# PhiFEM/phiFEM

Hardware: AMD Instinct MI355X
Metric: assembled+solved DoF/s, 3D Poisson phi-FEM (tag+assemble+solve) (higher is better)
Workload: dtype f64

## Files before the change

include/phifem_hip.h:

```cpp
#ifndef PHIFEM_HIP_H
#define PHIFEM_HIP_H

#include <stdint.h>

#ifdef __cplusplus
extern "C" {
#endif

typedef struct phx_mesh phx_mesh;
typedef struct phx_system phx_system;

enum phx_status {
  PHX_OK = 0,
  PHX_ERR_VALUE = -1,
  PHX_ERR_NOT_IMPLEMENTED = -2,
  PHX_ERR_HIP = -3,
  PHX_ERR_PARTITION = -4,
  PHX_ERR_CAPACITY = -5,
  PHX_ERR_BREAKDOWN = -6,
  PHX_ERR_TIMEOUT = -7
};

enum phx_loc { PHX_HOST = 0, PHX_DEVICE = 1 };

// ... 42 lines not shown
                            int32_t *c2f, int32_t *f2c, int64_t *nf);

int phx_mesh_create(int gdim, int cell_type, int64_t nv, const double *coords, int64_t nc,
                    const int32_t *cells, int device, phx_mesh **out);

int phx_mesh_create_box(int gdim, const double *lo, const double *hi, const int64_t *n,
                        const int64_t *offset, const int64_t *n_global, int device,
                        phx_mesh **out);

int phx_mesh_set_slab_faces(phx_mesh *m, int lower_is_cut, int upper_is_cut);
int phx_mesh_destroy(phx_mesh *m);
int phx_mesh_edge_count(phx_mesh *m, int64_t *ne);
int phx_mesh_counts(const phx_mesh *m, int64_t *counts);
int phx_mesh_get_array(phx_mesh *m, int which, void *out, int loc);
int phx_mesh_stream(phx_mesh *m, uint64_t *stream);
int phx_mesh_synchronize(phx_mesh *m);
int phx_mesh_set_stream(phx_mesh *m, uint64_t stream);
enum phx_option {
  PHX_OPT_PROFILE_SPMV = 1,
  PHX_OPT_HAS_EXTERIOR = 2,
  PHX_OPT_SPMV_XCD_GROUP = 3,
  PHX_OPT_PRECOND = 5,
  PHX_OPT_EXPORT_CSR = 7,
  PHX_OPT_STRUCTURED = 8,
  PHX_OPT_DETERMINISTIC = 9,
  PHX_OPT_EL_COARSE = 10,
  PHX_OPT_STENCIL_PLANE_ROWS = 11,
  PHX_OPT_P2_COARSE = 12,
  PHX_OPT_BOX_TAGS = 13,
  PHX_OPT_MULTILEVEL = 14,
  PHX_OPT_ELWD_COARSE = 15,
  PHX_OPT_BOX_FACET_ROWS = 16,
  PHX_OPT_RED_SPMV = 17,
  PHX_OPT_ALLOW_EMPTY = 6,
  PHX_OPT_SPMV_VALUE_INDEX = 4
};
int phx_set_option(phx_mesh *m, int option, int64_t value);
int phx_box_poisson_solve(int device, const int *L, const double *h, int f32, double *f_host);
int phx_box_dst_bench(int device, const int *L, int f32, int reps, double *out_us3);
int phx_dense_inverse(int device, int64_t n, double *a_host, int *singular);
int phx_event_pair_overhead(phx_mesh *m, double *seconds);
int phx_mesh_tag_histogram(const phx_mesh *m, int64_t *cells4, int64_t *facets7);

int phx_tag_cells(phx_mesh *m, int phi_kind, const double *phi, int loc, int detection_degree,
                  int single_layer_cut, int *warn_zero_denominator);

int phx_tag_facets(phx_mesh *m, int phi_kind, const double *phi, int loc, int detection_degree);

int phx_overwrite_tags(phx_mesh *m, int entity_is_facet, int64_t n, const int32_t *indices,
                       const int32_t *values);
int phx_set_tags(phx_mesh *m, int entity_is_facet, const int32_t *values, int loc);

int phx_mesh_selection(phx_mesh *m, int which, int32_t *out, int64_t *count);
int phx_integration_entities(phx_mesh *m, int which, int32_t *out, int64_t *n_pairs);

int phx_submesh_create(phx_mesh *m, phx_mesh **sub);
int phx_submesh_maps(phx_mesh *sub, int32_t *c_map, int32_t *v_map);

int phx_partition_cells(phx_mesh *m, int nparts, const int32_t *weights, int32_t *part, int loc);
int phx_partition_layout(phx_mesh *m, int nparts, const int32_t *part, int rank, int32_t *owner, uint8_t *flags, int loc);
int phx_submesh_create_from_flags(phx_mesh *m, const uint8_t *flags, int loc, phx_mesh **sub);

int phx_mesh_refine(phx_mesh *m, phx_mesh **fine);
int phx_prolongate(phx_mesh *coarse, phx_mesh *fine, int degree, int ncomp, const double *in, int loc_in,
                   double *out, int loc_out);
int phx_refine_tables(int cell_type, int32_t *children, int *nchild, double *p2_weights);
// ... 34 lines not shown
int phx_system_update_rhs(phx_system *s, const double *phi_h, const double *f_h, const double *g_h,
                          const double *u_D, int loc);
int phx_assemble_diffusion_wd(phx_mesh *m, double pen_coef, double stab_coef, double reaction, const double *kappa_h,
                              const double *phi_h, const double *f_h, const double *g_h, const double *u_D, int loc,
                              phx_system **out);
int phx_system_destroy(phx_system *s);
int phx_system_info(const phx_system *s, int64_t *info);
int phx_system_export(phx_system *s, int64_t *rowptr, int32_t *col, double *val, double *rhs,
                      int64_t *dof);
int phx_system_export_sell(phx_system *s, int64_t *slice_ptr, int32_t *col, double *val, int32_t *rows);

enum phx_method { PHX_BICGSTAB_JACOBI = 0 };
int phx_solve(phx_system *s, int method, double rtol, int64_t max_iter, double *x, int loc,
              double *stats);
int phx_solve_from(phx_system *s, int method, double rtol, int64_t max_iter, const double *x0, double *x, int loc,
                   double *stats);

int phx_krylov_attach(phx_system *s, double *work, double *scal, const uint8_t *own);
int phx_krylov_precond_active(const phx_system *s, int *active);
int phx_precond_local_bbox(phx_system *s, int64_t *out6);
int phx_precond_setup_global(phx_system *s, const int64_t *bbox6, int nranks, int rank, const int64_t *zb,
                             int64_t *ncol);
int phx_precond_set_carry_buffers(phx_system *s, double *send, double *recv);
int phx_precond_dist_info(const phx_system *s, int64_t *out4);
int phx_krylov_precond_disable(phx_system *s);
int phx_precond_info(phx_system *s, double *out);
int phx_multilevel_setup(phx_system *s);
int phx_coarse_info(phx_system *s, double *out);
int phx_coarse_export(phx_system *s, int32_t *node_of, double *ainv);
int phx_coarse_apply(phx_system *s, const double *in, double *out, double *gc, double *zc, int loc);
int phx_krylov_identity_loop(const phx_system *s, int *on);
int phx_krylov_reduced_loop(const phx_system *s, int *on);
int phx_krylov_reduced_io(phx_system *s, int which, double *host, int64_t count, int put);
int phx_krylov_phase(phx_system *s, int phase);
int phx_krylov_finish(phx_system *s, double *x, int loc);
int phx_krylov_profile(phx_system *s, int reset, double *avg_seconds, int64_t *count);
int phx_system_get_perm(phx_system *s, int32_t *perm, int32_t *dof_u, int32_t *dof_p, int loc);

typedef struct phx_comm phx_comm;
int phx_comm_unique_id(void *out128);
int phx_comm_create(int nranks, int rank, const void *uid128, int device, phx_comm **out);
int phx_comm_destroy(phx_comm *c);
int phx_comm_library(char *out, int64_t len);
int phx_comm_overlap(const phx_comm *c, int *out);
int phx_solve_distributed(phx_system *s, phx_comm *c, int npeers, const int *peers,
                          const int64_t *counts, const int64_t *const *idx, double rtol,
                          int64_t max_iter, double *x, int loc, double *stats);
int phx_halo_selftest(phx_system *s, phx_comm *c, int npeers, const int *peers,
                      const int64_t *counts, const int64_t *const *idx, double *vec);

int phx_spmv(phx_system *s, const double *x, double *y, int loc);
int phx_reference_nodes(int gdim, int degree, double *bary, int *n_nodes);
int phx_cell_errors(phx_mesh *m, int ncomp, int degree_h, const double *u_h, const double *u_ref,
                    int64_t ncells, const int32_t *cell_list, int loc, double *l2_local,
                    double *h10_local, double *norms);
int phx_estimate_poisson_wd(phx_mesh *m, int degree, const double *u, const double *p, const double *phi,
                            const double *f, const double *u_D, int loc_in, double *eta2_parts, int loc_out,
                            double *sums3);
int phx_mark_dorfler(phx_mesh *m, int64_t n, const double *eta2, int loc_in, double theta, uint8_t *marked,
                     int loc_out, int64_t *n_marked);
int phx_recover_gradient(phx_mesh *m, int degree, int ncomp, const double *u, int loc_u, const uint8_t *cell_mask,
                         int loc_mask, double *grad, double *eta2, int loc_out, double *sum);

int phx_spmv_bench(phx_system *s, int reps, double *out);

int phx_last_timings(const phx_mesh *m, double *t);
// ... 6 lines not shown
```

phifem_amd/_lib.py:

```python
import ctypes as C
import os

_HERE = os.path.dirname(os.path.abspath(__file__))
LIB_PATH = os.path.join(_HERE, "libphifem_hip.so")

if not os.path.exists(LIB_PATH):
    raise ImportError(
        f"{LIB_PATH} is missing: build it with `python -c 'import __graft_entry__ as g; g.build()'` "
        "(or `make -C phifem_amd/csrc`).  phifem_amd has no CPU fallback.")

if os.environ.get("PHIFEM_NO_TORCH", "") != "1":
    try:
        import torch
    except ImportError:
        pass

lib = C.CDLL(LIB_PATH)

HOST, DEVICE = 0, 1
TRIANGLE, QUADRILATERAL, TETRAHEDRON = 0, 1, 2
CELL_TYPES = {"triangle": TRIANGLE, "quadrilateral": QUADRILATERAL, "tetrahedron": TETRAHEDRON}
CELL_NAMES = {v: k for k, v in CELL_TYPES.items()}
PHI_NODAL_P1, PHI_POINTS, PHI_QUADRIC = 0, 1, 2
(OPT_PROFILE_SPMV, OPT_HAS_EXTERIOR, OPT_SPMV_XCD_GROUP, OPT_SPMV_VALUE_INDEX, OPT_PRECOND, OPT_ALLOW_EMPTY,
 OPT_EXPORT_CSR, OPT_STRUCTURED, OPT_DETERMINISTIC, OPT_EL_COARSE, OPT_STENCIL_PLANE_ROWS, OPT_P2_COARSE,
 OPT_BOX_TAGS, OPT_MULTILEVEL, OPT_ELWD_COARSE, OPT_BOX_FACET_ROWS, OPT_RED_SPMV) = (
    1, 2, 3, 4, 5, 6, 7, 8, 9, 10, 11, 12, 13, 14, 15, 16, 17)
(ARR_COORDS, ARR_CELLS, ARR_C2F, ARR_F2C, ARR_CELL_TAGS, ARR_FACET_TAGS, ARR_BFACETS, ARR_C2E,
 ARR_EDGES, ARR_PARENT_CELLS, ARR_CHILD_NODES) = range(11)

OK, ERR_VALUE, ERR_NOT_IMPLEMENTED, ERR_HIP, ERR_PARTITION, ERR_CAPACITY, ERR_BREAKDOWN, ERR_TIMEOUT = (
    0, -1, -2, -3, -4, -5, -6, -7)

_vp, _i, _i64, _d = C.c_void_p, C.c_int, C.c_int64, C.c_double
_pi, _pi64, _pd = C.POINTER(C.c_int), C.POINTER(C.c_int64), C.POINTER(C.c_double)

SIGNATURES = {
    "phx_version": ([], _i),
    "phx_last_error": ([], C.c_char_p),
    "phx_device_count": ([_pi], _i),
    "phx_pool_release": ([], _i),
    "phx_pool_stats": ([_pi64, _pi64], _i),
    "phx_detection_points": ([_i, _i, _i, _vp, _pi64], _i),
    "phx_levelset_points_count": ([_vp, _i, _pi64], _i),
    "phx_levelset_eval_points": ([_vp, _i, _vp, _i, _vp], _i),
    "phx_detection_points_physical": ([_vp, _i, _vp], _i),
    "phx_lagrange_nodes": ([_i, _i, _vp, _pi64], _i),
    "phx_lagrange_tabulate": ([_i, _i, _i64, _vp, _vp], _i),
    "phx_levelset_eval_points_deg": ([_vp, _i, _i, _vp, _i, _vp], _i),
    "phx_lagrange_dof_points": ([_vp, _i, _vp], _i),
    "phx_topology_build_host": ([_i, _i64, _i64, _vp, _vp, _vp, _pi64], _i),
    "phx_mesh_create": ([_i, _i, _i64, _vp, _i64, _vp, _i, C.POINTER(_vp)], _i),
    "phx_mesh_create_box": ([_i, _vp, _vp, _vp, _vp, _vp, _i, C.POINTER(_vp)], _i),
    "phx_mesh_set_slab_faces": ([_vp, _i, _i], _i),
    "phx_mesh_destroy": ([_vp], _i),
    "phx_mesh_counts": ([_vp, _pi64], _i),
    "phx_mesh_edge_count": ([_vp, _pi64], _i),
    "phx_mesh_get_array": ([_vp, _i, _vp, _i], _i),
    "phx_mesh_stream": ([_vp, C.POINTER(C.c_uint64)], _i),
    "phx_mesh_synchronize": ([_vp], _i),
# ... 41 lines not shown
    "phx_mesh_refine": ([_vp, C.POINTER(_vp)], _i),
    "phx_prolongate": ([_vp, _vp, _i, _i, _vp, _i, _vp, _i], _i),
    "phx_restrict": ([_vp, _vp, _i, _i, _vp, _i, _vp, _i], _i),
    "phx_refine_tables": ([_i, _vp, _pi, _vp], _i),
    "phx_mesh_refine_marked": ([_vp, _vp, _vp, _i, C.POINTER(_vp), _pi64], _i),
    "phx_locate_points": ([_vp, _i64, _vp, _i, _d, _vp, _vp, _i], _i),
    "phx_eval_points": ([_vp, _i, _i, _vp, _i, _i64, _vp, _vp, _i, _i, _d, _vp, _vp, _i], _i),
    "phx_locator_info": ([_vp, _pi64], _i),
    "phx_locate_timings": ([_vp, _pd], _i),
    "phx_assemble_poisson_wd": ([_vp, _d, _d, _vp, _vp, _vp, _i, C.POINTER(_vp)], _i),
    "phx_box_facet_tables": ([_i, _vp, _d, _pi, _vp, _vp, _vp, _vp], _i),
    "phx_assemble_poisson_wd_p2": ([_vp, _d, _d, _vp, _i, _vp, _vp, _i, C.POINTER(_vp)], _i),
    "phx_assemble_poisson_sd": ([_vp, _d, _i, _vp, _i, _vp, _i, C.POINTER(_vp)], _i),
    "phx_assemble_poisson_flux": ([_vp, _vp, _i, _i, _vp, _vp, _vp, _i, C.POINTER(_vp)], _i),
    "phx_assemble_elasticity_if": ([_vp, _vp, _vp, _vp, _vp, _vp, _i64, _i, C.POINTER(_vp)], _i),
    "phx_assemble_elasticity_wd": ([_vp, _vp, _vp, _vp, _vp, _i, C.POINTER(_vp)], _i),
    "phx_assemble_reaction_wd": ([_vp, _d, _d, _d, _vp, _vp, _vp, _vp, _i, C.POINTER(_vp)], _i),
    "phx_system_update_rhs": ([_vp, _vp, _vp, _vp, _vp, _i], _i),
    "phx_assemble_diffusion_wd": ([_vp, _d, _d, _d, _vp, _vp, _vp, _vp, _vp, _i, C.POINTER(_vp)], _i),
    "phx_reference_nodes": ([_i, _i, _vp, C.POINTER(C.c_int)], _i),
    "phx_cell_errors": ([_vp, _i, _i, _vp, _vp, _i64, _vp, _i, _vp, _vp, _pd], _i),
    "phx_estimate_poisson_wd": ([_vp, _i, _vp, _vp, _vp, _vp, _vp, _i, _vp, _i, _pd], _i),
    "phx_mark_dorfler": ([_vp, _i64, _vp, _i, _d, _vp, _i, _pi64], _i),
    "phx_recover_gradient": ([_vp, _i, _i, _vp, _i, _vp, _i, _vp, _vp, _i, _pd], _i),
    "phx_system_destroy": ([_vp], _i),
    "phx_system_info": ([_vp, _pi64], _i),
    "phx_system_export": ([_vp, _vp, _vp, _vp, _vp, _vp], _i),
    "phx_system_export_sell": ([_vp, _vp, _vp, _vp, _vp], _i),
    "phx_solve": ([_vp, _i, _d, _i64, _vp, _i, _pd], _i),
    "phx_solve_from": ([_vp, _i, _d, _i64, _vp, _vp, _i, _pd], _i),
    "phx_krylov_identity_loop": ([_vp, C.POINTER(C.c_int)], _i),
    "phx_krylov_reduced_loop": ([_vp, C.POINTER(C.c_int)], _i),
    "phx_krylov_reduced_io": ([_vp, _i, _vp, _i64, _i], _i),
    "phx_spmv": ([_vp, _vp, _vp, _i], _i),
    "phx_spmv_bench": ([_vp, _i, _pd], _i),
    "phx_last_timings": ([_vp, _pd], _i),
}
for _name, (_args, _res) in SIGNATURES.items():
    _fn = getattr(lib, _name)
    _fn.argtypes = _args
    _fn.restype = _res


class PartitionError(ValueError):
    """The reference's facet sets overlap: dolfinx MeshTags would reject the duplicated entities."""


def check(rc):
    if rc == OK:
        return
    msg = lib.phx_last_error().decode()
    if rc == ERR_VALUE:
        raise ValueError(msg)
    if rc == ERR_NOT_IMPLEMENTED:
        raise NotImplementedError(msg)
    if rc == ERR_PARTITION:
        raise PartitionError(msg)
    if rc == ERR_CAPACITY:
        raise MemoryError(msg)
    if rc == ERR_BREAKDOWN:
        raise ArithmeticError(msg)
    if rc == ERR_TIMEOUT:
        raise TimeoutError(msg)
    raise RuntimeError(msg)


# ... 22 lines not shown
```

phifem_amd/csrc/phx_common.h:

```cpp
#pragma once
#include <hip/hip_runtime.h>
#include <stdint.h>
#include <stdio.h>
#include <string>
#include <vector>

#include "../../include/phifem_hip.h"
#include "phx_switches.h"

#define PHX_MAX_PTS 40
#define PHX_MAX_VPC 4

void phx_set_error(const char *fmt, ...);

hipError_t phx_pool_malloc(void **p, size_t bytes);
hipError_t phx_pool_free(void *p);
void phx_pool_trim(void);
template <typename T>
static inline hipError_t phx_malloc(T **p, size_t bytes) { return phx_pool_malloc((void **)p, bytes); }
static inline hipError_t phx_free(void *p) { return phx_pool_free(p); }

#define PHX_HIP(expr)                                                                       \
  do {                                                                                      \
    hipError_t e_ = (expr);                                                                 \
// ... 94 lines not shown
  bool sel_counts_valid = false;
  int64_t sel_total[2] = {0, 0};
  int32_t *sel_counts_cut = nullptr;
  bool sel_cut_valid = false;
  uint8_t *act_in = nullptr, *act_cut = nullptr;
  bool act_valid = false;
  int64_t *ent_buf[2] = {nullptr, nullptr};
  int64_t ent_count[2] = {0, 0};
  bool have_entities = false;
  bool is_submesh = false;
  int32_t *c_map_h = nullptr, *v_map_h = nullptr;
  bool on_box_lattice = false;
  int32_t *v2lat = nullptr;
  int32_t *lat2v = nullptr;
  double timings[8] = {0, 0, 0, 0, 0, 0, 0, 0};
  struct phx_locator *locator = nullptr;
  int rect_checked = 0;
  double loc_timings[3] = {0, 0, 0};
  bool own_stream = true;
  int profile_spmv = 0;
  int spmv_xcd_group = 0;
  int64_t stencil_plane_rows = 32768;
  int spmv_value_index = 1;
  int precond = 1;
  int has_exterior_override = -1;
  std::vector<hipEvent_t> prof_ev[2];
  int prof_used[2] = {0, 0}, prof_seen[2] = {0, 0};
  double *scal_h = nullptr;
  int export_csr = 0;
  int structured = 1;
  int box_tags = 1;
  int box_facet_rows = 1;
  int red_spmv = 1;
  int allow_empty = 0;
  int el_coarse = -1;
  int p2_coarse = 0;
  int elwd_coarse = 0;
  int deterministic = 0;
  int multilevel = 0;
  phx_mesh *inner = nullptr;
  int32_t *in_cmap = nullptr;
  int32_t *in_fmap = nullptr;
};

struct phx_p2_lattice {
  int64_t n[3];
  int64_t F[3];
  int64_t nv;
  int64_t base[8];
  int64_t ext[7][3];
};
__host__ __device__ __forceinline__ int phx_p2_edge_class(int a, int b, int c) {
  const int nd = a + b + c;
  return nd == 1 ? (a ? 0 : (b ? 1 : 2)) : (nd == 2 ? (!c ? 3 : (!b ? 4 : 5)) : 6);
}
__host__ __device__ __forceinline__ int64_t phx_p2_entity_of_fine(const phx_p2_lattice &L, int64_t I, int64_t J, int64_t K) {
  const int a = (int)(I & 1), b = (int)(J & 1), c = (int)(K & 1);
  const int64_t i = I >> 1, j = J >> 1, k = K >> 1;
  if (!(a | b | c)) return i + (L.n[0] + 1) * (j + (L.n[1] + 1) * k);
  const int cls = phx_p2_edge_class(a, b, c);
  return L.nv + L.base[cls] + i + L.ext[cls][0] * (j + L.ext[cls][1] * k);
}
__host__ __device__ __forceinline__ void phx_p2_fine_of_entity(const phx_p2_lattice &L, int64_t e, int64_t *q) {
  if (e < L.nv) {
    const int64_t n0 = L.n[0] + 1, n1 = L.n[1] + 1, r = e / n0;
    q[0] = 2 * (e - r * n0); q[1] = 2 * (r % n1); q[2] = 2 * (r / n1);
// ... 164 lines not shown
```

phifem_amd/csrc/phx_dst_wave.inc.hip:

```cpp
typedef unsigned phx_v2u __attribute__((ext_vector_type(2)));
#define PHX_BUF_OOB 0x80000000u

__device__ __forceinline__ __amdgpu_buffer_rsrc_t buf_rsrc(const void *p, uint32_t bytes) {
  return __builtin_amdgcn_make_buffer_rsrc(const_cast<void *>(p), 0, (int)bytes, 0x00020000);
}
__device__ __forceinline__ double buf_ld_f64(__amdgpu_buffer_rsrc_t rs, uint32_t off) {
  return __builtin_bit_cast(double, __builtin_amdgcn_raw_buffer_load_b64(rs, (int)off, 0, 0));
}
__device__ __forceinline__ int32_t buf_ld_i32(__amdgpu_buffer_rsrc_t rs, uint32_t off) {
  return (int32_t)__builtin_amdgcn_raw_buffer_load_b32(rs, (int)off, 0, 0);
}
__device__ __forceinline__ void buf_st_f64(double v, __amdgpu_buffer_rsrc_t rs, uint32_t off) {
  __builtin_amdgcn_raw_buffer_store_b64(__builtin_bit_cast(phx_v2u, v), rs, (int)off, 0, 0);
}

template <int LL> struct WaveShape {
  static constexpr int TP = LL / 8;
  static constexpr int SLOT = TP <= 32 ? 32 : 64;
  static constexpr int PAIRS = LL >= 512 ? 4 : 8;
  static constexpr int NTHR = PAIRS * SLOT;
  static constexpr int W = 2 * PAIRS;
  static constexpr int RSTEP = NTHR / W;
  static constexpr int H = LL / 2;
  static constexpr int ZL = ZLEN(LL);
// ... 97 lines not shown
    const int pr = tid / S::SLOT, t = tid % S::SLOT;
    if (2 * pr < ncols && t < S::TP) dst_core<double, true, LL>(zs + pr * S::ZL, nullptr, P, t, true, tw);
  }
  __syncthreads();
  {
    constexpr int NS = (len + S::RSTEP - 1) / S::RSTEP;
    const int zr = ZP(row0 + 1);
    const uint32_t offs = colok ? (uint32_t)(tcol * 8 + row0 * pitch8) : PHX_BUF_OOB;
    const uint32_t ds = (uint32_t)(row0 - srlo);
    double v[NS];
#pragma unroll
    for (int i = 0; i < NS; ++i) v[i] = wcol[2 * (zr + i * ZS)];
#pragma unroll
    for (int i = 0; i < NS; ++i) {
      const bool ok = ds + (uint32_t)(i * S::RSTEP) <= sspan;
      buf_st_f64(v[i], rs, ok ? offs + (uint32_t)i * dstep : PHX_BUF_OOB);
    }
  }
}

template <int LL, int IO, bool SC>
__global__ void __launch_bounds__(WaveShape<LL>::NTHR)
k_dst_xw(BoxGrid g, DstPlan P, double *__restrict__ G, const int32_t *__restrict__ gmap,
         const double *__restrict__ vin, double *__restrict__ vout, const double *__restrict__ dscale,
         const uint8_t *__restrict__ line_any, uint32_t vec_bytes) {
  using S = WaveShape<LL>;
  extern __shared__ double2 zs_raw[];
  C2<double> *zs = reinterpret_cast<C2<double> *>(zs_raw);
  constexpr int TP = S::TP;
  constexpr int ZS = TP + TP / 8;
  const int tid = (int)threadIdx.x;
  const int pr = tid / S::SLOT, t = tid % S::SLOT;
  const int nlines = g.m[1] * g.m[2];
  if (IO != 0 && line_any) {
    const int lane = tid & 63, l = (int)blockIdx.x * S::PAIRS * 2 + lane;
    const bool mine = lane < 2 * S::PAIRS && l < nlines && line_any[l] != 0;
    if (__ballot(mine) == 0) return;
  }
  const int line0 = ((int)blockIdx.x * S::PAIRS + pr) * 2;
  const bool live = line0 < nlines && t < TP;
  C2<double> *w = zs + pr * S::ZL;
  const C2<double> *tw;
  const double *sn;
  WaveTables<LL> tab;
  const uint32_t lat = (uint32_t)nlines * (uint32_t)g.pitch;
  const __amdgpu_buffer_rsrc_t rsG = buf_rsrc(G, lat * 8u);
  const __amdgpu_buffer_rsrc_t rsM = buf_rsrc(gmap, IO != 0 ? lat * 4u : 0u);
  const __amdgpu_buffer_rsrc_t rsV = buf_rsrc(IO == 1 ? (const void *)vin : (const void *)vout, IO != 0 ? vec_bytes : 0u);
  const __amdgpu_buffer_rsrc_t rsS = buf_rsrc(dscale, SC ? vec_bytes : 0u);
  bool has[2] = {false, false};
  uint32_t base[2] = {0, 0};
  double va[4], vb[4], ua[4], ub[4], sj[4];
  if (live) {
#pragma unroll
    for (int c = 0; c < 2; ++c) {
      const int l = line0 + c;
      has[c] = l < nlines && !(IO != 0 && line_any && !line_any[l]);
      base[c] = (uint32_t)l * (uint32_t)g.pitch;
    }
    const double *sng = P.sintab;
    const uint32_t ea = base[0] + (uint32_t)t, eb = base[1] + (uint32_t)t;
    const uint32_t fa = base[0] + (uint32_t)(LL - 2 - t), fb = base[1] + (uint32_t)(LL - 2 - t);
    if (IO == 1) {
      int32_t qa[4], qb[4], pa[4], pb[4];
#pragma unroll
      for (int i = 0; i < 4; ++i) {
        qa[i] = buf_ld_i32(rsM, has[0] ? (ea + (uint32_t)(i * TP)) * 4u : PHX_BUF_OOB);
        qb[i] = buf_ld_i32(rsM, has[1] ? (eb + (uint32_t)(i * TP)) * 4u : PHX_BUF_OOB);
        pa[i] = buf_ld_i32(rsM, has[0] ? (fa - (uint32_t)(i * TP)) * 4u : PHX_BUF_OOB);
        pb[i] = buf_ld_i32(rsM, has[1] ? (fb - (uint32_t)(i * TP)) * 4u : PHX_BUF_OOB);
        sj[i] = sng[1 + t + i * TP];
      }
#pragma unroll
      for (int i = 0; i < 4; ++i) {
        const uint32_t oqa = has[0] ? (uint32_t)qa[i] << 3 : PHX_BUF_OOB, oqb = has[1] ? (uint32_t)qb[i] << 3 : PHX_BUF_OOB;
        const uint32_t opa = has[0] ? (uint32_t)pa[i] << 3 : PHX_BUF_OOB, opb = has[1] ? (uint32_t)pb[i] << 3 : PHX_BUF_OOB;
        va[i] = buf_ld_f64(rsV, oqa); vb[i] = buf_ld_f64(rsV, oqb);
        ua[i] = buf_ld_f64(rsV, opa); ub[i] = buf_ld_f64(rsV, opb);
        if (SC) {
          va[i] *= buf_ld_f64(rsS, oqa); vb[i] *= buf_ld_f64(rsS, oqb);
          ua[i] *= buf_ld_f64(rsS, opa); ub[i] *= buf_ld_f64(rsS, opb);
        }
      }
    } else {
#pragma unroll
      for (int i = 0; i < 4; ++i) {
        va[i] = buf_ld_f64(rsG, has[0] ? (ea + (uint32_t)(i * TP)) * 8u : PHX_BUF_OOB);
        vb[i] = buf_ld_f64(rsG, has[1] ? (eb + (uint32_t)(i * TP)) * 8u : PHX_BUF_OOB);
        ua[i] = buf_ld_f64(rsG, has[0] ? (fa - (uint32_t)(i * TP)) * 8u : PHX_BUF_OOB);
        ub[i] = buf_ld_f64(rsG, has[1] ? (fb - (uint32_t)(i * TP)) * 8u : PHX_BUF_OOB);
// ... 80 lines not shown
```

phifem_amd/csrc/phx_mesh.hip:

```cpp
#include "phx_prim.h"
#include <stdarg.h>
#include <string.h>

#include <algorithm>
#include <atomic>
#include <mutex>
#include <unordered_map>
#include <vector>

#include "phx_common.h"
#include "phx_select.h"

static thread_local char g_err[1024] = "";

void phx_set_error(const char *fmt, ...) {
  va_list ap;
  va_start(ap, fmt);
  vsnprintf(g_err, sizeof(g_err), fmt, ap);
  va_end(ap);
}

#include <map>
#include <mutex>
#include <unordered_map>
// ... 1014 lines not shown
  PHX_HIP(phx_malloc(&m->edges, sizeof(int32_t) * 2 * (size_t)m->ne));
  k_edge_vertices<<<grid, block, 0, m->stream>>>(m->nc, m->ci.nvpc, m->cell_type == PHX_TETRAHEDRON ? 6 : 3,
                                                 m->cell_type == PHX_TETRAHEDRON ? 1 : 0, m->cells,
                                                 m->c2e, m->edges);
  PHX_HIP(hipGetLastError());
  PHX_HIP(hipStreamSynchronize(m->stream));
  return PHX_OK;
}

extern "C" int phx_mesh_edge_count(phx_mesh *m, int64_t *ne) {
  PHX_HIP(hipSetDevice(m->device));
  PHX_CHECK(phx_mesh_build_edges(m));
  *ne = m->ne;
  return PHX_OK;
}

extern "C" int phx_mesh_destroy(phx_mesh *m) {
  if (!m) return PHX_OK;
  (void)hipSetDevice(m->device);
  (void)hipDeviceSynchronize();
  void *ptrs[] = {m->x, m->cells, m->c2f, m->f2c, m->bfacets, m->bfacet_ids, m->cell_tags,
                  m->facet_tags, m->ent_buf[0], m->ent_buf[1], m->facet_exempt, m->v2c_ptr, m->v2c_idx,
                  m->edges, m->c2e_is_alias ? nullptr : (void *)m->c2e};
  for (void *p : ptrs) (void)phx_free(p);
  free(m->c_map_h); free(m->v_map_h);
  (void)phx_free(m->v2lat); (void)phx_free(m->lat2v);
  (void)phx_free(m->in_cmap); (void)phx_free(m->in_fmap);
  (void)phx_free(m->rm_parent); (void)phx_free(m->rm_child); (void)phx_free(m->rm_mid);
  (void)phx_free(m->rs_ptr); (void)phx_free(m->rs_idx);
  if (m->inner) { phx_mesh_destroy(m->inner); m->inner = nullptr; }
  phx_locator_destroy(m->locator);
  if (m->scal_h) (void)hipHostFree(m->scal_h);
  for (auto &pe : m->prof_ev) for (auto &e : pe) (void)hipEventDestroy(e);
  for (int w = 0; w < 2; ++w) (void)phx_free(m->sel_counts[w]);
  (void)phx_free(m->sel_counts_cut);
  (void)phx_free(m->act_in); (void)phx_free(m->act_cut);
  if (m->ev0) (void)hipEventDestroy(m->ev0);
  if (m->ev1) (void)hipEventDestroy(m->ev1);
  if (m->stream && m->own_stream) (void)hipStreamDestroy(m->stream);
  delete m;
  return PHX_OK;
}

extern "C" int phx_mesh_counts(const phx_mesh *m, int64_t *counts) {
  counts[0] = m->gdim; counts[1] = m->cell_type; counts[2] = m->nv;
  counts[3] = m->nc; counts[4] = m->nf; counts[5] = m->nbf;
  return PHX_OK;
}

struct RbArgs { const uint8_t *src[8]; int bytes[8], off[8], n; };
__global__ void k_rb_pack(RbArgs a, uint8_t *__restrict__ out) {
  for (int i = 0; i < a.n; ++i)
    for (int b = threadIdx.x; b < a.bytes[i]; b += blockDim.x) out[a.off[i] + b] = a.src[i][b];
}
int phx_read_back(hipStream_t st, const phx_rb_item *items, int n) {
  PHX_REQUIRE(n >= 1 && n <= 8, PHX_ERR_VALUE, "read-back of %d items", n);
  struct Stage { uint8_t *dev = nullptr, *pin = nullptr; };
  static std::mutex mu;
  static std::map<std::pair<int, hipStream_t>, Stage> stages;
  int dev = 0;
  PHX_HIP(hipGetDevice(&dev));
  Stage sg;
  {
    std::lock_guard<std::mutex> lk(mu);
    Stage &ref = stages[{dev, st}];
    if (!ref.dev) {
// ... 27 lines not shown
  return PHX_OK;
}

extern "C" int phx_mesh_stream(phx_mesh *m, uint64_t *stream) {
  *stream = (uint64_t)(uintptr_t)m->stream;
  return PHX_OK;
}

extern "C" int phx_mesh_set_stream(phx_mesh *m, uint64_t stream) {
  PHX_HIP(hipSetDevice(m->device));
  PHX_HIP(hipStreamSynchronize(m->stream));
  if (m->own_stream) PHX_HIP(hipStreamDestroy(m->stream));
  m->stream = (hipStream_t)(uintptr_t)stream;
  m->own_stream = false;
  if (m->inner) m->inner->stream = m->stream;
  return PHX_OK;
}

extern "C" int phx_set_option(phx_mesh *m, int option, int64_t value) {
  if (m->inner) PHX_CHECK(phx_set_option(m->inner, option, value));
  switch (option) {
    case PHX_OPT_PROFILE_SPMV:
      PHX_REQUIRE(value >= 0 && value <= 1024, PHX_ERR_VALUE, "SpMV profiling stride out of range");
      m->profile_spmv = (int)value;
      return PHX_OK;
    case PHX_OPT_HAS_EXTERIOR: m->has_exterior_override = (int)value; return PHX_OK;
    case PHX_OPT_SPMV_VALUE_INDEX: m->spmv_value_index = value != 0; return PHX_OK;
    case PHX_OPT_ALLOW_EMPTY: m->allow_empty = value != 0; return PHX_OK;
    case PHX_OPT_EXPORT_CSR: m->export_csr = value != 0; return PHX_OK;
    case PHX_OPT_STRUCTURED: m->structured = value != 0; return PHX_OK;
    case PHX_OPT_BOX_TAGS: m->box_tags = value != 0; return PHX_OK;
    case PHX_OPT_BOX_FACET_ROWS: m->box_facet_rows = value != 0; return PHX_OK;
    case PHX_OPT_RED_SPMV: m->red_spmv = value != 0; return PHX_OK;
    case PHX_OPT_DETERMINISTIC: m->deterministic = value != 0; return PHX_OK;
    case PHX_OPT_MULTILEVEL: m->multilevel = value != 0; return PHX_OK;
    case PHX_OPT_EL_COARSE:
      PHX_REQUIRE(value == -1 || value == 0 || (value >= 5 && value <= 4096), PHX_ERR_VALUE, "coarse ratio %lld: -1, 0 or >= 5", (long long)value);
      m->el_coarse = (int)value;
      return PHX_OK;
    case PHX_OPT_P2_COARSE:
      PHX_REQUIRE(value == -1 || value == 0 || (value >= 5 && value <= 4096), PHX_ERR_VALUE, "coarse ratio %lld: -1, 0 or >= 5", (long long)value);
      m->p2_coarse = (int)value;
      return PHX_OK;
    case PHX_OPT_ELWD_COARSE:
      PHX_REQUIRE(value == -1 || value == 0 || (value >= 5 && value <= 4096), PHX_ERR_VALUE, "coarse ratio %lld: -1, 0 or >= 5", (long long)value);
      m->elwd_coarse = (int)value;
      return PHX_OK;
    case PHX_OPT_PRECOND:
      PHX_REQUIRE(value >= 0 && value <= 2, PHX_ERR_VALUE, "unknown preconditioner %lld", (long long)value);
      m->precond = (int)value;
      return PHX_OK;
    case PHX_OPT_SPMV_XCD_GROUP:
      PHX_REQUIRE(value >= 0 && value < (1 << 24), PHX_ERR_VALUE, "XCD group size out of range");
      m->spmv_xcd_group = (int)value;
      return PHX_OK;
    case PHX_OPT_STENCIL_PLANE_ROWS:
      PHX_REQUIRE(value >= 0, PHX_ERR_VALUE, "rows per plane out of range");
      m->stencil_plane_rows = value;
      return PHX_OK;
    default: phx_set_error("unknown option %d", option); return PHX_ERR_VALUE;
  }
}

extern "C" int phx_mesh_tag_histogram(const phx_mesh *m, int64_t *cells4, int64_t *facets7) {
  if (cells4) for (int i = 0; i < 4; ++i) cells4[i] = m->tag_hist[i];
  if (facets7) for (int i = 0; i < 7; ++i) facets7[i] = m->ftag_hist[i];
// ... 67 lines not shown
```

phifem_amd/csrc/phx_precond.inc.hip:

```cpp
#include <limits.h>
#include <math.h>

#include <map>
#include <tuple>

#define PHX_PRECOND_MARGIN 4

struct DstPlan {
  int L = 0, nstage = 0, pairs = 0, tp = 0;
  int slot = 0;
  int wave = 0;
  int radix[8], pw[8], tws[8];
  int scr = 0;
  int tab_off = 0;
  int lds_elems = 0;
  double2 *tw = nullptr;
  double *sintab = nullptr;
  float2 *tw_f = nullptr;
  float *sintab_f = nullptr;
};

static std::map<std::pair<int, int>, DstPlan> g_dst_plans;

static int dst_pick_length(int64_t need) {
// ... 1191 lines not shown
static int box_red_maps(phx_system *s) {
  phx_box_precond *bp = s->precond;
  if (bp->red_map[0]) return PHX_OK;
  hipStream_t st = s->mesh->stream;
  const int64_t n = s->n, tot = bp->g.plane * bp->g.m[2], nlines = (int64_t)bp->g.m[1] * bp->g.m[2];
  PHX_REQUIRE(tot > 0 && bp->line_iv, PHX_ERR_VALUE, "reduced loop: empty lattice");
  DevTemps tmp(st);
  int32_t *bidx = nullptr;
  uint8_t *cols = nullptr;
  PHX_HIP(tmp.alloc(&bidx, sizeof(int32_t) * (size_t)n));
  PHX_HIP(tmp.alloc(&cols, (size_t)n));
  for (int k = 0; k < 2; ++k) {
    PHX_HIP(phx_malloc(&bp->red_map[k], sizeof(int32_t) * (size_t)tot));
    PHX_HIP(phx_malloc(&bp->red_any[k], (size_t)nlines));
    PHX_HIP(phx_malloc(&bp->red_iv[k], sizeof(int2) * (size_t)bp->g.m[2]));
  }
  PHX_HIP(hipMemsetAsync(bidx, 0xff, sizeof(int32_t) * (size_t)n, st));
  PHX_HIP(hipMemsetAsync(cols, 0, (size_t)n, st));
  const dim3 block(256);
  k_red_bidx<<<dim3((unsigned)phx_div_up(s->n_sell_rows, 256)), block, 0, st>>>(s->n_sell_rows, s->sell_rows, bidx);
  k_red_cols<<<dim3((unsigned)std::max<int64_t>(1, std::min<int64_t>(phx_div_up(s->sell_nnz, 256), 4096))), block, 0, st>>>(
      s->sell_nnz, n, s->sell_col, cols);
  k_red_maps<<<dim3((unsigned)std::min<int64_t>(phx_div_up(tot, 256), 8192)), block, 0, st>>>(tot, bp->gmap, bidx, cols,
                                                                                             bp->red_map[0], bp->red_map[1]);
  for (int k = 0; k < 2; ++k) {
    k_line_any<<<dim3((unsigned)phx_div_up(nlines * 64, 256)), block, 0, st>>>(bp->g, bp->red_map[k], bp->red_any[k]);
    k_line_intervals<<<dim3((unsigned)bp->g.m[2]), dim3(64), 0, st>>>(bp->g.m[1], bp->g.m[2], bp->red_any[k], bp->red_iv[k]);
  }
  PHX_HIP(hipGetLastError());
  PHX_HIP(hipStreamSynchronize(st));
  return PHX_OK;
}

static int box_precond_apply_red(phx_system *s, const double *vin, double *vout) {
  phx_box_precond *bp = s->precond;
  hipStream_t st = s->mesh->stream;
  int32_t *gmap = bp->gmap;
  uint8_t *any = bp->line_any;
  int2 *iv = bp->line_iv;
  const int64_t nvec = bp->nvec;
  bp->rowskip = true;
  bp->gmap = bp->red_map[0]; bp->line_any = bp->red_any[0]; bp->line_iv = bp->red_iv[0]; bp->line_iv_out = bp->red_iv[1];
  bp->nvec = s->n_sell_rows;
  int rc = box_pass_x<1>(bp, st, vin, nullptr);
  if (rc == PHX_OK) rc = box_solve_middle(bp, st, s);
  bp->gmap = bp->red_map[1]; bp->line_any = bp->red_any[1]; bp->nvec = s->n;
  if (rc == PHX_OK) rc = box_pass_x<2>(bp, st, nullptr, vout);
  bp->gmap = gmap; bp->line_any = any; bp->line_iv = iv; bp->line_iv_out = nullptr; bp->nvec = nvec;
  bp->rowskip = false;
  return rc;
}

extern "C" int phx_box_poisson_solve(int device, const int *L, const double *h, int f32, double *f_host) {
  PHX_HIP(hipSetDevice(device));
  for (int a = 0; a < 3; ++a)
    PHX_REQUIRE(dst_pick_length(L[a]) == L[a] || (a == 2 && L[a] >= 2 && L[a] <= 1025), PHX_ERR_VALUE,
                "L[%d] = %d is not a supported transform length", a, L[a]);
  phx_box_precond *bp = new phx_box_precond();
  const double c[3] = {h[1] * h[2] / h[0], h[0] * h[2] / h[1], h[0] * h[1] / h[2]};
  int rc = box_grid_setup(bp, device, L, c, f32 != 0);
  if (rc != PHX_OK) { box_precond_free(bp); return rc; }
  const BoxGrid &g = bp->g;
  const size_t tot = (size_t)(g.plane * g.m[2]);
  std::vector<double> tmp(tot, 0.0);
  for (int64_t z = 0; z < g.m[2]; ++z)
    for (int64_t y = 0; y < g.m[1]; ++y)
      memcpy(&tmp[z * g.plane + y * g.pitch], &f_host[(z * g.m[1] + y) * g.m[0]], sizeof(double) * (size_t)g.m[0]);
  std::vector<float> tmpf;
  if (f32) { tmpf.resize(tot); for (size_t i = 0; i < tot; ++i) tmpf[i] = (float)tmp[i]; }
  const void *src = f32 ? (const void *)tmpf.data() : (const void *)tmp.data();
  const size_t bytes = (f32 ? sizeof(float) : sizeof(double)) * tot;
  hipStream_t st = nullptr;
  if (hipMemcpy(bp->G, src, bytes, hipMemcpyHostToDevice) != hipSuccess) { box_precond_free(bp); return PHX_ERR_HIP; }
  rc = box_pass_x<0>(bp, st, nullptr, nullptr);
  if (rc == PHX_OK) rc = box_solve_middle(bp, st);
  if (rc == PHX_OK) rc = box_pass_x<0>(bp, st, nullptr, nullptr);
  if (rc == PHX_OK && hipDeviceSynchronize() != hipSuccess) rc = PHX_ERR_HIP;
  void *dst = f32 ? (void *)tmpf.data() : (void *)tmp.data();
  if (rc == PHX_OK && hipMemcpy(dst, bp->G, bytes, hipMemcpyDeviceToHost) != hipSuccess) rc = PHX_ERR_HIP;
  if (rc == PHX_OK) {
// ... 45 lines not shown
```

phifem_amd/csrc/phx_solve.hip:

```cpp
#include "phx_prim.h"
#include <math.h>
#include <stdlib.h>
#include <string.h>

#include <algorithm>
#include <memory>
#include <type_traits>
#include <vector>

#include "phx_common.h"
#include "phx_select.h"

#define SELL_C 64
#define SELL_S 16
static const int64_t SELL_WINDOW = (int64_t)1 << 40;
#ifdef PHX_SPMV_NT
#define NT_LOAD(p) __builtin_nontemporal_load(p)
#else
#define NT_LOAD(p) (*(p))
#endif
#define NSLOT 64
#define SLOT_STRIDE 8
#define P_OFF 16
#define PHX_SCAL_DOUBLES (P_OFF + 2 * 8 * NSLOT * SLOT_STRIDE)
// ... 2319 lines not shown
  return PHX_OK;
}

extern "C" int phx_krylov_precond_active(const phx_system *s, int *active) {
  *active = kr_hats_apart(s) ? 1 : 0;
  return PHX_OK;
}

extern "C" int phx_krylov_identity_loop(const phx_system *s, int *on) {
  *on = s->kr_ident_used ? 1 : 0;
  return PHX_OK;
}

extern "C" int phx_krylov_reduced_loop(const phx_system *s, int *on) {
  *on = s->kr_red_used ? 1 : 0;
  return PHX_OK;
}

extern "C" int phx_krylov_reduced_io(phx_system *s, int which, double *host, int64_t count, int put) {
  PHX_HIP(hipSetDevice(s->mesh->device));
  PHX_REQUIRE(s->kr_red_used, PHX_ERR_VALUE, "the reduced loop is not in force for this system");
  PHX_REQUIRE(which >= 0 && which <= 10, PHX_ERR_VALUE, "reduced-loop buffer %d: 0 .. 10", which);
  const KrVecs V = kr_vecs(s);
  const int64_t m = s->nslices * SELL_S;
  double *dev = which <= 7 ? s->kr_red + which * m : which == 8 ? V.phat : which == 9 ? V.shat : kr_scal(s);
  const int64_t len = which <= 6 ? m : which <= 9 ? s->n : (int64_t)PHX_SCAL_DOUBLES;
  PHX_REQUIRE(count == len, PHX_ERR_VALUE, "reduced-loop buffer %d holds %lld doubles, not %lld", which, (long long)len, (long long)count);
  PHX_HIP(hipStreamSynchronize(s->mesh->stream));
  if (put) PHX_HIP(hipMemcpy(dev, host, sizeof(double) * (size_t)len, hipMemcpyHostToDevice));
  else PHX_HIP(hipMemcpy(host, dev, sizeof(double) * (size_t)len, hipMemcpyDeviceToHost));
  return PHX_OK;
}

extern "C" int phx_krylov_precond_disable(phx_system *s) {
  if (s->precond_state == 1) {
    PHX_HIP(hipSetDevice(s->mesh->device));
    PHX_HIP(hipStreamSynchronize(s->mesh->stream));
    phx_box_precond_destroy(s->precond);
    s->precond = nullptr;
  }
  s->precond_state = -1;
  return PHX_OK;
}

extern "C" int phx_krylov_attach(phx_system *s, double *work, double *scal, const uint8_t *own) {
  s->kr_work = work;
  s->kr_scal = scal;
  s->own = own;
  return PHX_OK;
}

extern "C" int phx_event_pair_overhead(phx_mesh *m, double *seconds) {
  PHX_HIP(hipSetDevice(m->device));
  const int reps = 32;
  hipEvent_t ev[2 * reps];
  for (auto &e : ev) PHX_HIP(hipEventCreate(&e));
  for (int i = 0; i < reps; ++i) {
    PHX_HIP(hipEventRecord(ev[2 * i], m->stream));
    PHX_HIP(hipEventRecord(ev[2 * i + 1], m->stream));
  }
  PHX_HIP(hipEventSynchronize(ev[2 * reps - 1]));
  double tot = 0.0;
  for (int i = 0; i < reps; ++i) {
    float ms = 0.f;
    PHX_HIP(hipEventElapsedTime(&ms, ev[2 * i], ev[2 * i + 1]));
    tot += ms;
// ... 81 lines not shown
      PHX_HIP(hipMemcpyAsync(tmp, in, nb, hipMemcpyHostToDevice, st));
      PHX_HIP(hipMemcpyAsync(tmp + s->n, out, nb, hipMemcpyHostToDevice, st));
      din = tmp; dout = tmp + s->n;
    }
    const hipMemcpyKind k = dev ? hipMemcpyDeviceToDevice : hipMemcpyDeviceToHost;
    PHX_CHECK(coarse_restrict(s, c, din));
    if (gc) PHX_HIP(hipMemcpyAsync(gc, c->gc, ncb, k, st));
    PHX_CHECK(coarse_apply_end(s, c, dout));
    if (zc) PHX_HIP(hipMemcpyAsync(zc, c->zc, ncb, k, st));
    if (!dev) PHX_HIP(hipMemcpyAsync(out, dout, nb, hipMemcpyDeviceToHost, st));
    return PHX_OK;
  };
  const int rc = run();
  const bool synced = hipStreamSynchronize(st) == hipSuccess;
  (void)phx_free(tmp);
  if (rc != PHX_OK) return rc;
  PHX_REQUIRE(synced, PHX_ERR_HIP, "phx_coarse_apply: the stream failed to synchronise");
  return PHX_OK;
}

#include "phx_dist.inc.hip"

static int kr_drive(phx_system *s, const KrDist *d, double rtol, int64_t max_iter, double *x_out, int loc,
                    double *stats) {
  phx_mesh *m = s->mesh;
  hipStream_t st = m->stream;
  const int mode = d ? 1 : 0;
  double *S = kr_scal(s);
  const KrVecs V = kr_vecs(s);
  const bool ident = s->kr_ident_used;
  const bool red = s->kr_red_used;
  const bool pc = d ? d->pc_all : kr_precond_on_u_block(s);
  const double bb = s->scal_h[S_BB];
  auto read_head = [&](const char *what) -> int {
    PHX_HIP(hipMemcpyAsync(s->scal_h, S, sizeof(double) * 16, hipMemcpyDeviceToHost, st));
    if (d) return stream_sync_watchdog(st, what);
    PHX_HIP(hipStreamSynchronize(st));
    return PHX_OK;
  };
  auto allreduce = [&](int lo, int hi) -> int { return d ? allreduce_R(s, d->c, lo, hi) : PHX_OK; };
  auto precond = [&](int ph, int ph_exact, int ph_restrict, int ph_add) -> int {
    PHX_CHECK(kr_phase(s, ph, mode, 0));
    if (d && d->exact) { PHX_CHECK(allgather_carries(s, d->c)); PHX_CHECK(kr_phase(s, ph_exact, mode, 0)); }
    if (d && d->coarse) {
      PHX_CHECK(kr_phase(s, ph_restrict, mode, 0));
      PHX_CHECK(allreduce_sum(d->c, s->cc->gc, (size_t)s->cc->nc, st));
      PHX_CHECK(kr_phase(s, ph_add, mode, 0));
    }
    return PHX_OK;
  };
  auto spmv = [&](int ph, int ph_inner, int ph_halo, double *in, int par) -> int {
    if (d && d->overlap) {
      PHX_CHECK(halo_begin(s, d->c, *d->H, in, true));
      PHX_CHECK(kr_phase(s, ph_inner, mode, par));
      PHX_CHECK(halo_end(s, d->c, *d->H, in, true));
      return kr_phase(s, ph_halo, mode, par);
    }
    if (d) PHX_CHECK(halo_exchange(s, d->c, *d->H, in));
    return kr_phase(s, ph, mode, par);
  };
  int64_t it = 0, spmvs = 0, next_check = pc ? 2 : 8, last_check = 0;
  double relres = bb == 0.0 ? 0.0 : 1.0, last_relres = 1.0;
  int rc = PHX_OK;
  int verifications = 0;
  bool skip = red && bb != 0.0 && s->scal_h[S_RR] == 0.0;
  if (skip) relres = 0.0;
  for (;;) {
    while (bb != 0.0 && it < max_iter && !skip) {
      const int par = d ? 0 : (int)(it & 1);
      if (red) {
        PHX_CHECK(kr_phase(s, KR_RED_PRECOND_P, mode, par));
        PHX_CHECK(kr_phase(s, KR_RED_SPMV_P, mode, par));
        PHX_CHECK(kr_phase(s, KR_RED_UPDATE_S, mode, par));
        PHX_CHECK(kr_phase(s, KR_RED_PRECOND_S, mode, par));
        PHX_CHECK(kr_phase(s, KR_RED_SPMV_S, mode, par));
        PHX_CHECK(kr_phase(s, KR_RED_UPDATE_XRP, mode, par));
      } else {
        PHX_CHECK(precond(KR_PRECOND_P, KR_EXACT_P, KR_CC_RESTRICT_P, KR_CC_ADD_P));
        PHX_CHECK(spmv(ident ? KR_ID_SPMV_P : KR_SPMV_P, KR_SPMV_P_INNER, KR_SPMV_P_HALO, V.phat, par));
        PHX_CHECK(allreduce(R_RV, R_RV + 1));
        PHX_CHECK(kr_phase(s, ident ? KR_ID_UPDATE_S : KR_UPDATE_S, mode, par));
        PHX_CHECK(precond(KR_PRECOND_S, KR_EXACT_S, KR_CC_RESTRICT_S, KR_CC_ADD_S));
        PHX_CHECK(spmv(ident ? KR_ID_SPMV_S : KR_SPMV_S, KR_SPMV_S_INNER, KR_SPMV_S_HALO, V.shat, par));
        PHX_CHECK(allreduce(R_TS, R_TT + 1));
        PHX_CHECK(kr_phase(s, ident ? KR_ID_UPDATE_XRP : KR_UPDATE_XR, mode, par));
        PHX_CHECK(allreduce(R_RHO, R_RR + 1));
      }
      spmvs += 2;
      ++it;
      if (it >= next_check || it == max_iter) {
        if (!d) k_reduce_slots<<<1, 64, 0, st>>>(S, par, R_RHO, 2, 0);
        PHX_CHECK(read_head("convergence check of the distributed solve"));
        const double rr = s->scal_h[R_OFF + R_RR];
        const double omega = s->scal_h[S_OMEGA];
        relres = sqrt(rr / bb);
        if (!(rr == rr) || !(fabs(rr) <= 1.0e300) || !(omega == omega)) {
          phx_set_error("BiCGStab breakdown at iteration %lld (omega=%g rr=%g)", (long long)it, omega, rr);
          rc = PHX_ERR_BREAKDOWN;
          break;
        }
        if (relres <= rtol) break;
        int64_t step = pc ? 2 : 8;
        if (pc && relres < last_relres && relres > 0.0) {
          const double rate = log(last_relres / relres) / (double)(it - last_check);
          const double remaining = log(relres / rtol) / rate;
          step = std::max<int64_t>(2, std::min<int64_t>(12, (int64_t)(0.5 * remaining)));
          step &= ~(int64_t)1;
        }
        last_check = it;
        last_relres = relres;
        next_check = it + step;
      }
      if (!ident) PHX_CHECK(kr_phase(s, KR_UPDATE_P, mode, par));
    }
    if (red && rc == PHX_OK && bb != 0.0) PHX_CHECK(kr_phase(s, KR_RED_FORM_X, mode, 0));
    if (rc != PHX_OK || bb == 0.0 || !(relres <= rtol)) break;
    if (d) PHX_CHECK(halo_exchange(s, d->c, *d->H, V.y));
    else PHX_HIP(hipMemsetAsync(S + P_OFF, 0, sizeof(double) * (PHX_SCAL_DOUBLES - P_OFF), st));
    PHX_CHECK(kr_phase(s, KR_TRUE_SPMV, mode, 0));
    PHX_CHECK(kr_phase(s, KR_TRUE_RESIDUAL, mode, 0));
    PHX_CHECK(allreduce(R_RR, R_RR + 1));
    PHX_CHECK(read_head("true-residual check of the distributed solve"));
    spmvs += 1;
    const double rr_true = s->scal_h[R_OFF + R_RR];
    if (!(rr_true == rr_true)) { phx_set_error("non-finite true residual"); rc = PHX_ERR_BREAKDOWN; break; }
    relres = sqrt(rr_true / bb);
    if (relres <= rtol || ++verifications > 8 || it >= max_iter) break;
    PHX_CHECK(kr_phase(s, red ? KR_RED_RESTART : KR_RESTART, mode, d ? 0 : (int)(it & 1)));
    skip = false;
    last_relres = relres;
    last_check = it;
    next_check = it + 2;
  }
  PHX_CHECK(phx_krylov_finish(s, x_out, loc));
  PHX_CHECK(phx_end_timing(m, 3));
  double pavg = 0.0;
  int pcount = 0;
  PHX_CHECK(prof_collect(s, &pavg, &pcount));
  if (stats) {
    stats[0] = (double)it;
    stats[1] = relres;
    stats[2] = m->timings[3];
    stats[3] = (double)spmvs;
    stats[4] = pavg;
    stats[5] = (double)pcount;
    stats[6] = relres <= rtol ? 1.0 : 0.0;
    stats[7] = d ? (d->pc_all ? 1.0 : 0.0) : s->scal_h[S_RESTARTS];
// ... 75 lines not shown
```

Before: 125.7 million.

## Overlap first half of reduced preconditioner with host convergence-check sync

At each convergence check in the reduced BiCGStab loop, the first half of the box preconditioner (x pass and first y pass) on p is enqueued after the residual head copy. The host then waits on an event instead of synchronizing the whole stream, and the next iteration runs only the remaining passes. This is meant to keep the GPU busy during the host round-trip. The DST wave kernel also applies the line_any skip mask to all pass types, not only the input/output x passes. A timing probe for the preconditioner x pass is added as well. The risks are wasted preconditioner work on the final converged check and correctness depending on p being final at check time.

New measurement: 125.6 million. No clear change (-0.1%).

```diff
diff --git a/include/phifem_hip.h b/include/phifem_hip.h
--- a/include/phifem_hip.h
+++ b/include/phifem_hip.h
@@ -98,6 +98,7 @@
   PHX_OPT_ELWD_COARSE = 15,
   PHX_OPT_BOX_FACET_ROWS = 16,
   PHX_OPT_RED_SPMV = 17,
+  PHX_OPT_RED_LOOKAHEAD = 18,
   PHX_OPT_ALLOW_EMPTY = 6,
   PHX_OPT_SPMV_VALUE_INDEX = 4
 };
@@ -198,6 +199,7 @@
 int phx_krylov_identity_loop(const phx_system *s, int *on);
 int phx_krylov_reduced_loop(const phx_system *s, int *on);
 int phx_krylov_reduced_io(phx_system *s, int which, double *host, int64_t count, int put);
+int phx_box_precond_x_bound(phx_system *s, int reps, int flush_mb, double *out);
 int phx_krylov_phase(phx_system *s, int phase);
 int phx_krylov_finish(phx_system *s, double *x, int loc);
 int phx_krylov_profile(phx_system *s, int reset, double *avg_seconds, int64_t *count);
diff --git a/phifem_amd/_lib.py b/phifem_amd/_lib.py
--- a/phifem_amd/_lib.py
+++ b/phifem_amd/_lib.py
@@ -24,8 +24,8 @@
 PHI_NODAL_P1, PHI_POINTS, PHI_QUADRIC = 0, 1, 2
 (OPT_PROFILE_SPMV, OPT_HAS_EXTERIOR, OPT_SPMV_XCD_GROUP, OPT_SPMV_VALUE_INDEX, OPT_PRECOND, OPT_ALLOW_EMPTY,
  OPT_EXPORT_CSR, OPT_STRUCTURED, OPT_DETERMINISTIC, OPT_EL_COARSE, OPT_STENCIL_PLANE_ROWS, OPT_P2_COARSE,
- OPT_BOX_TAGS, OPT_MULTILEVEL, OPT_ELWD_COARSE, OPT_BOX_FACET_ROWS, OPT_RED_SPMV) = (
-    1, 2, 3, 4, 5, 6, 7, 8, 9, 10, 11, 12, 13, 14, 15, 16, 17)
+ OPT_BOX_TAGS, OPT_MULTILEVEL, OPT_ELWD_COARSE, OPT_BOX_FACET_ROWS, OPT_RED_SPMV, OPT_RED_LOOKAHEAD) = (
+    1, 2, 3, 4, 5, 6, 7, 8, 9, 10, 11, 12, 13, 14, 15, 16, 17, 18)
 (ARR_COORDS, ARR_CELLS, ARR_C2F, ARR_F2C, ARR_CELL_TAGS, ARR_FACET_TAGS, ARR_BFACETS, ARR_C2E,
  ARR_EDGES, ARR_PARENT_CELLS, ARR_CHILD_NODES) = range(11)
 
@@ -133,6 +133,7 @@
     "phx_krylov_identity_loop": ([_vp, C.POINTER(C.c_int)], _i),
     "phx_krylov_reduced_loop": ([_vp, C.POINTER(C.c_int)], _i),
     "phx_krylov_reduced_io": ([_vp, _i, _vp, _i64, _i], _i),
+    "phx_box_precond_x_bound": ([_vp, _i, _i, _pd], _i),
     "phx_spmv": ([_vp, _vp, _vp, _i], _i),
     "phx_spmv_bench": ([_vp, _i, _pd], _i),
     "phx_last_timings": ([_vp, _pd], _i),
diff --git a/phifem_amd/csrc/phx_common.h b/phifem_amd/csrc/phx_common.h
--- a/phifem_amd/csrc/phx_common.h
+++ b/phifem_amd/csrc/phx_common.h
@@ -150,6 +150,8 @@
   int box_tags = 1;
   int box_facet_rows = 1;
   int red_spmv = 1;
+  int red_lookahead = 1;
+  hipEvent_t check_ev = nullptr;
   int allow_empty = 0;
   int el_coarse = -1;
   int p2_coarse = 0;
diff --git a/phifem_amd/csrc/phx_dst_wave.inc.hip b/phifem_amd/csrc/phx_dst_wave.inc.hip
--- a/phifem_amd/csrc/phx_dst_wave.inc.hip
+++ b/phifem_amd/csrc/phx_dst_wave.inc.hip
@@ -153,7 +153,7 @@
   const int tid = (int)threadIdx.x;
   const int pr = tid / S::SLOT, t = tid % S::SLOT;
   const int nlines = g.m[1] * g.m[2];
-  if (IO != 0 && line_any) {
+  if (line_any) {
     const int lane = tid & 63, l = (int)blockIdx.x * S::PAIRS * 2 + lane;
     const bool mine = lane < 2 * S::PAIRS && l < nlines && line_any[l] != 0;
     if (__ballot(mine) == 0) return;
@@ -176,7 +176,7 @@
 #pragma unroll
     for (int c = 0; c < 2; ++c) {
       const int l = line0 + c;
-      has[c] = l < nlines && !(IO != 0 && line_any && !line_any[l]);
+      has[c] = l < nlines && !(line_any && !line_any[l]);
       base[c] = (uint32_t)l * (uint32_t)g.pitch;
     }
     const double *sng = P.sintab;
diff --git a/phifem_amd/csrc/phx_mesh.hip b/phifem_amd/csrc/phx_mesh.hip
--- a/phifem_amd/csrc/phx_mesh.hip
+++ b/phifem_amd/csrc/phx_mesh.hip
@@ -1070,6 +1070,7 @@
   phx_locator_destroy(m->locator);
   if (m->scal_h) (void)hipHostFree(m->scal_h);
   for (auto &pe : m->prof_ev) for (auto &e : pe) (void)hipEventDestroy(e);
+  if (m->check_ev) (void)hipEventDestroy(m->check_ev);
   for (int w = 0; w < 2; ++w) (void)phx_free(m->sel_counts[w]);
   (void)phx_free(m->sel_counts_cut);
   (void)phx_free(m->act_in); (void)phx_free(m->act_cut);
@@ -1163,6 +1164,7 @@
     case PHX_OPT_BOX_TAGS: m->box_tags = value != 0; return PHX_OK;
     case PHX_OPT_BOX_FACET_ROWS: m->box_facet_rows = value != 0; return PHX_OK;
     case PHX_OPT_RED_SPMV: m->red_spmv = value != 0; return PHX_OK;
+    case PHX_OPT_RED_LOOKAHEAD: m->red_lookahead = value != 0; return PHX_OK;
     case PHX_OPT_DETERMINISTIC: m->deterministic = value != 0; return PHX_OK;
     case PHX_OPT_MULTILEVEL: m->multilevel = value != 0; return PHX_OK;
     case PHX_OPT_EL_COARSE:
diff --git a/phifem_amd/csrc/phx_precond.inc.hip b/phifem_amd/csrc/phx_precond.inc.hip
--- a/phifem_amd/csrc/phx_precond.inc.hip
+++ b/phifem_amd/csrc/phx_precond.inc.hip
@@ -1247,7 +1247,7 @@
   return PHX_OK;
 }
 
-static int box_precond_apply_red(phx_system *s, const double *vin, double *vout) {
+static int box_precond_apply_red(phx_system *s, const double *vin, double *vout, int part = 0) {
   phx_box_precond *bp = s->precond;
   hipStream_t st = s->mesh->stream;
   int32_t *gmap = bp->gmap;
@@ -1257,10 +1257,17 @@
   bp->rowskip = true;
   bp->gmap = bp->red_map[0]; bp->line_any = bp->red_any[0]; bp->line_iv = bp->red_iv[0]; bp->line_iv_out = bp->red_iv[1];
   bp->nvec = s->n_sell_rows;
-  int rc = box_pass_x<1>(bp, st, vin, nullptr);
-  if (rc == PHX_OK) rc = box_solve_middle(bp, st, s);
-  bp->gmap = bp->red_map[1]; bp->line_any = bp->red_any[1]; bp->nvec = s->n;
-  if (rc == PHX_OK) rc = box_pass_x<2>(bp, st, nullptr, vout);
+  int rc = PHX_OK;
+  if (part != 2 && part != 4) {
+    rc = box_pass_x<1>(bp, st, vin, nullptr);
+    if (rc == PHX_OK && part != 3) rc = bp->f32 ? box_pass_y_t<float>(bp, st, s, 1) : box_pass_y_t<double>(bp, st, s, 1);
+  }
+  if (part != 1 && part != 3) {
+    if (rc == PHX_OK && part != 4) rc = bp->f32 ? box_pass_z_t<float>(bp, st) : box_pass_z_t<double>(bp, st);
+    if (rc == PHX_OK && part != 4) rc = bp->f32 ? box_pass_y_t<float>(bp, st, s, 2) : box_pass_y_t<double>(bp, st, s, 2);
+    bp->gmap = bp->red_map[1]; bp->line_any = bp->red_any[1]; bp->nvec = s->n;
+    if (rc == PHX_OK) rc = box_pass_x<2>(bp, st, nullptr, vout);
+  }
   bp->gmap = gmap; bp->line_any = any; bp->line_iv = iv; bp->line_iv_out = nullptr; bp->nvec = nvec;
   bp->rowskip = false;
   return rc;
diff --git a/phifem_amd/csrc/phx_solve.hip b/phifem_amd/csrc/phx_solve.hip
--- a/phifem_amd/csrc/phx_solve.hip
+++ b/phifem_amd/csrc/phx_solve.hip
@@ -2375,6 +2375,49 @@
   return PHX_OK;
 }
 
+extern "C" int phx_box_precond_x_bound(phx_system *s, int reps, int flush_mb, double *out) {
+  PHX_HIP(hipSetDevice(s->mesh->device));
+  PHX_REQUIRE(s->kr_red_used && s->precond_state == 1 && s->precond->red_map[0] && !s->precond->f32, PHX_ERR_VALUE,
+              "the reduced loop is not in force for this system");
+  PHX_REQUIRE(reps >= 2 && reps <= 1000 && flush_mb >= 0 && flush_mb <= 4096, PHX_ERR_VALUE, "reps 2 .. 1000, flush_mb 0 .. 4096");
+  phx_box_precond *bp = s->precond;
+  PHX_REQUIRE(dst_wave_fast(bp->g, bp->plan[0], s->n), PHX_ERR_VALUE, "the x passes of this lattice do not run the wave kernels");
+  hipStream_t st = s->mesh->stream;
+  DevTemps tmp(st);
+  char *flush = nullptr;
+  const size_t fb = (size_t)flush_mb << 20;
+  if (fb) PHX_HIP(tmp.alloc(&flush, fb));
+  hipEvent_t e0, e1;
+  PHX_HIP(hipEventCreate(&e0));
+  PHX_HIP(hipEventCreate(&e1));
+  uint8_t *any = bp->line_any;
+  int rc = PHX_OK;
+  for (int v = 0; v < 4 && rc == PHX_OK; ++v) {
+    const int k = v / 2;
+    double sum = 0.0, sq = 0.0;
+    for (int r = -2; r < reps && rc == PHX_OK; ++r) {
+      if (fb && hipMemsetAsync(flush, r & 1, fb, st) != hipSuccess) rc = PHX_ERR_HIP;
+      (void)hipEventRecord(e0, st);
+      if (v % 2 == 1) {
+        bp->line_any = bp->red_any[k];
+        rc = box_pass_x<0>(bp, st, nullptr, nullptr);
+        bp->line_any = any;
+      } else {
+        rc = box_precond_apply_red(s, kr_red_vecs(s).p, kr_vecs(s).phat, 3 + k);
+      }
+      (void)hipEventRecord(e1, st);
+      if (hipEventSynchronize(e1) != hipSuccess) rc = PHX_ERR_HIP;
+      float ms = 0.f;
+      (void)hipEventElapsedTime(&ms, e0, e1);
+      if (r >= 0) { sum += 1e3 * ms; sq += 1e6 * (double)ms * ms; }
+    }
+    out[2 * v] = sum / reps;
+    out[2 * v + 1] = sqrt(std::max(0.0, sq / reps - out[2 * v] * out[2 * v]));
+  }
+  (void)hipEventDestroy(e0); (void)hipEventDestroy(e1);
+  return rc;
+}
+
 extern "C" int phx_krylov_precond_disable(phx_system *s) {
   if (s->precond_state == 1) {
     PHX_HIP(hipSetDevice(s->mesh->device));
@@ -2522,9 +2565,18 @@
   const bool red = s->kr_red_used;
   const bool pc = d ? d->pc_all : kr_precond_on_u_block(s);
   const double bb = s->scal_h[S_BB];
-  auto read_head = [&](const char *what) -> int {
+  bool half_ahead = false;
+  auto read_head = [&](const char *what, bool ahead = false) -> int {
     PHX_HIP(hipMemcpyAsync(s->scal_h, S, sizeof(double) * 16, hipMemcpyDeviceToHost, st));
     if (d) return stream_sync_watchdog(st, what);
+    if (ahead) {
+      if (!m->check_ev) PHX_HIP(hipEventCreateWithFlags(&m->check_ev, hipEventDisableTiming));
+      PHX_HIP(hipEventRecord(m->check_ev, st));
+      PHX_CHECK(box_precond_apply_red(s, kr_red_vecs(s).p, V.phat, 1));
+      half_ahead = true;
+      PHX_HIP(hipEventSynchronize(m->check_ev));
+      return PHX_OK;
+    }
     PHX_HIP(hipStreamSynchronize(st));
     return PHX_OK;
   };
@@ -2559,7 +2611,9 @@
     while (bb != 0.0 && it < max_iter && !skip) {
       const int par = d ? 0 : (int)(it & 1);
       if (red) {
-        PHX_CHECK(kr_phase(s, KR_RED_PRECOND_P, mode, par));
+        if (half_ahead) PHX_CHECK(box_precond_apply_red(s, kr_red_vecs(s).p, V.phat, 2));
+        else PHX_CHECK(kr_phase(s, KR_RED_PRECOND_P, mode, par));
+        half_ahead = false;
         PHX_CHECK(kr_phase(s, KR_RED_SPMV_P, mode, par));
         PHX_CHECK(kr_phase(s, KR_RED_UPDATE_S, mode, par));
         PHX_CHECK(kr_phase(s, KR_RED_PRECOND_S, mode, par));
@@ -2580,7 +2634,7 @@
       ++it;
       if (it >= next_check || it == max_iter) {
         if (!d) k_reduce_slots<<<1, 64, 0, st>>>(S, par, R_RHO, 2, 0);
-        PHX_CHECK(read_head("convergence check of the distributed solve"));
+        PHX_CHECK(read_head("convergence check of the distributed solve", red && m->red_lookahead != 0 && it < max_iter));
         const double rr = s->scal_h[R_OFF + R_RR];
         const double omega = s->scal_h[S_OMEGA];
         relres = sqrt(rr / bb);
@@ -2603,6 +2657,7 @@
       }
       if (!ident) PHX_CHECK(kr_phase(s, KR_UPDATE_P, mode, par));
     }
+    half_ahead = false;
     if (red && rc == PHX_OK && bb != 0.0) PHX_CHECK(kr_phase(s, KR_RED_FORM_X, mode, 0));
     if (rc != PHX_OK || bb == 0.0 || !(relres <= rtol)) break;
     if (d) PHX_CHECK(halo_exchange(s, d->c, *d->H, V.y));
```
